# hilbertw/stereo_matching

Measured on AMD Instinct MI355X. Metric: Mpixel-disparities/s, 8-path SGM @ KITTI 1242×375 D=128; 1→8 GPU scaling, higher is better.
Workload: dtype f32; 1 GPU; config2: KITTI 1242x375 D=128, census 9x7 + Hamming cost + 8-path SGM + WTA/uniqueness/sub-pixel, left view (V=1), 1 pair per GPU; width=1242, height=375, max_disp=128, views=1, post_filter=False, lk_refine=False, sky_detect=False, launch=eager, pairs_per_gpu=1, global_batch=1, parallelism=1 pair on 1 GPU (single process: no process group, no gather)

## Files before the change

### stereo_matching_amd/csrc/sgm_cost.hip

```cpp
#include "sgm_device.h"

namespace sgm {


__device__ __forceinline__ int reflect101(int i, int n) {
    if (n == 1) return 0;
    i = i < 0 ? -i : i;
    return i >= n ? 2 * n - 2 - i : i;
}

constexpr int CT_TW = 64, CT_TH = 16, CT_RPT = CT_TH / 4;

template <int HH, int HWW>
__global__ __launch_bounds__(256) void census_kernel(const uint8_t *__restrict__ src0,
                                                     const uint8_t *__restrict__ src1, int rpitch,
                                                     int step, int H, int W, int blur,
                                                     uint64_t *__restrict__ ct0,
                                                     uint64_t *__restrict__ ct1) {
    const bool second = __builtin_amdgcn_workgroup_id_z() != 0;
    const uint8_t *__restrict__ src = second ? src1 : src0;
    uint64_t *__restrict__ ct = second ? ct1 : ct0;
    constexpr int TR = CT_TH + 2 * HH, TC = CT_TW + 2 * HWW;
    constexpr int RR = TR + 2, RC = TC + 2;
    constexpr int RAW_IT = (RR * RC + 255) / 256;
    __shared__ uint8_t tile[TR][TC];
    __shared__ uint8_t raw[RR][RC];
    const int x0 = bid_x() * CT_TW, y0 = bid_y() * CT_TH;
    const int t = tid_x();
    if (blur) {
        const int ylo = y0 - HH > 0 ? y0 - HH : 0, xlo = x0 - HWW > 0 ? x0 - HWW : 0;
        uint8_t v[RAW_IT];
#pragma unroll
        for (int u = 0; u < RAW_IT; ++u) {
            const int idx = u * 256 + t;
            const int ry = idx / RC, rx = idx - ry * RC;
            const int y = reflect101(clampi(ylo - 1 + ry, -1, H), H);
            const int x = reflect101(clampi(xlo - 1 + rx, -1, W), W);
            v[u] = idx < RR * RC ? src[(size_t)y * rpitch + (size_t)x * step] : 0;
        }
#pragma unroll
        for (int u = 0; u < RAW_IT; ++u) {
            const int idx = u * 256 + t;
            if (idx < RR * RC) (&raw[0][0])[idx] = v[u];
        }
        __syncthreads();
        for (int idx = t; idx < TR * TC; idx += 256) {
            const int ty = idx / TC, tx = idx - ty * TC;
            const int ry = clampi(y0 + ty - HH, 0, H - 1) - ylo;
            const int rx = clampi(x0 + tx - HWW, 0, W - 1) - xlo;
            constexpr int ky[3] = {70, 116, 70};
            int acc = 0;
#pragma unroll
            for (int r = 0; r < 3; ++r) {
                const uint8_t *row = &raw[ry + r][rx];
                acc += ky[r] * (82 * row[0] + 93 * row[1] + 82 * row[2]);
            }
            const int b = (acc + (1 << 15)) >> 16;
            tile[ty][tx] = (uint8_t)(b > 255 ? 255 : b);
        }
    } else {
        for (int idx = t; idx < TR * TC; idx += 256) {
            const int ty = idx / TC, tx = idx - ty * TC;
            const int y = clampi(y0 + ty - HH, 0, H - 1), x = clampi(x0 + tx - HWW, 0, W - 1);
            tile[ty][tx] = src[(size_t)y * rpitch + (size_t)x * step];
        }
    }
    __syncthreads();
    const int tx = t & 63, r0 = wave_id() * CT_RPT;
    constexpr int NB = (2 * HH + 1) * (2 * HWW + 1) - 1;
    static_assert(NB <= 64, "census word");
    constexpr int NHI = NB > 32 ? NB - 32 : 0;
    int c[CT_RPT];
#pragma unroll
    for (int p = 0; p < CT_RPT; ++p) c[p] = tile[r0 + p + HH][tx + HWW];
    unsigned hi[CT_RPT], lo[CT_RPT];
#pragma unroll
    for (int p = 0; p < CT_RPT; ++p) hi[p] = lo[p] = 0;
#pragma unroll
    for (int rr = 0; rr < CT_RPT + 2 * HH; ++rr) {
        int b[2 * HWW + 1];
#pragma unroll
        for (int dj = 0; dj <= 2 * HWW; ++dj) b[dj] = tile[r0 + rr][tx + dj];
#pragma unroll
        for (int p = 0; p < CT_RPT; ++p) {
            const int di = rr - p;
            if (di < 0 || di > 2 * HH) continue;
#pragma unroll
            for (int dj = 0; dj <= 2 * HWW; ++dj) {
                if (di == HH && dj == HWW) continue;
                const int k = di * (2 * HWW + 1) + dj - (di * (2 * HWW + 1) + dj > HH * (2 * HWW + 1) + HWW ? 1 : 0);
                const unsigned x = (unsigned)(c[p] - b[dj]);
                if (k < NHI) hi[p] = (hi[p] << 1) | (x >> 31);
                else lo[p] = (lo[p] << 1) | (x >> 31);
            }
        }
    }
    const int x = x0 + tx;
#pragma unroll
    for (int p = 0; p < CT_RPT; ++p) {
        const int y = y0 + r0 + p;
        if (y < H && x < W) ct[(size_t)y * W + x] = ((uint64_t)hi[p] << 32) | lo[p];
    }
}

hipError_t launch_census(const uint8_t *src, int pitch, Geom g, int blur, uint64_t *ct,
                         hipStream_t st, bool bm_rows, const uint8_t *src2, uint64_t *ct2) {
    dim3 grid((g.W + CT_TW - 1) / CT_TW, (g.H + CT_TH - 1) / CT_TH, src2 ? 2 : 1);
    const int rpitch = bm_rows ? pitch : pitch * g.scale;
    if (g.scale == 1)
        census_kernel<3, 4><<<grid, 256, 0, st>>>(src, src2, rpitch, 1, g.H, g.W, blur, ct, ct2);
    else
        census_kernel<1, 2><<<grid, 256, 0, st>>>(src, src2, rpitch, 2, g.H, g.W, blur, ct, ct2);
    return hipGetLastError();
}


__global__ __launch_bounds__(256) void ct_shift_kernel(const uint64_t *__restrict__ ctl,
                                                       const uint64_t *__restrict__ ctr,
                                                       uint64_t *__restrict__ ctl_s,
                                                       uint64_t *__restrict__ ctr_s, int W, int k) {
    const bool right = __builtin_amdgcn_workgroup_id_z() != 0;
    const uint64_t *__restrict__ src = right ? ctr : ctl;
    uint64_t *__restrict__ dst = right ? ctr_s : ctl_s;
    const int x = bid_x() * 256 + tid_x();
    if (dst == nullptr || x >= W) return;
    const size_t row = (size_t)bid_y() * W;
    const int xs = right ? (x - k > 0 ? x - k : 0) : (x + k < W - 1 ? x + k : W - 1);
    dst[row + x] = src[row + xs];
}

hipError_t launch_ct_shift(const uint64_t *ctl, const uint64_t *ctr, uint64_t *ctl_s, uint64_t *ctr_s,
                           int k, Geom g, hipStream_t st) {
    ct_shift_kernel<<<dim3((g.W + 255) / 256, g.H, 2), 256, 0, st>>>(ctl, ctr, ctl_s, ctr_s, g.W, k);
    return hipGetLastError();
}


constexpr int COSTH_MAX_LDS = 64 * 1024;

__device__ __forceinline__ void costh_store(float v, float *p) { __builtin_nontemporal_store(v, p); }
constexpr int COSTH_U = 8;

__host__ __device__ constexpr int costh_pad(int D, int scale) { return D / scale + 2 * COSTH_U; }

template <int VIEW, int WIN, bool SKY, bool FILTER, bool UNI, int DC = 0, int CK = 0>
__device__ __forceinline__ void cost_h_body(const uint64_t *__restrict__ ctl,
                                            const uint64_t *__restrict__ ctr,
                                            const uint8_t *__restrict__ sky, int sky_pitch, int H,
                                            int W, int D, int scale, int R,
                                            float *__restrict__ out, int blk, unsigned char *smem,
                                            int ck_ns = 0) {
    static_assert(CK == 0 || (WIN == 5 && FILTER), "checkpoints of the 5-wide filter");
    const int P = costh_pad(D, scale), RS = W + 2 * P;
    constexpr int NS = UNI ? 1 : 2;
    uint64_t *sl = reinterpret_cast<uint64_t *>(smem);
    uint64_t *sr = sl + (UNI ? 0 : (size_t)R * RS);
    uint8_t *ss = reinterpret_cast<uint8_t *>(sl + (size_t)NS * R * RS);
    const int row0 = blk * R;
    for (int idx = tid_x(); idx < R * RS; idx += R * D) {
        const int r = idx / RS, jp = idx - r * RS, i = row0 + r;
        const int j = clampi(jp - P, 0, W - 1);
        if (i < H) {
            if (!UNI || VIEW == 1) sl[idx] = ctl[(size_t)i * W + j];
            if (!UNI || VIEW == 0) sr[idx] = ctr[(size_t)i * W + j];
            if (SKY) ss[idx] = sky[(size_t)i * sky_pitch + j];
        }
    }
    __syncthreads();
    const int r = UNI ? uniform(tid_x() / D) : tid_x() / D, d = tid_x() - r * D;
    const int i = row0 + r;
    if (i >= H) return;
    const int ds = d / scale;
    const uint64_t *cl = sl + (size_t)r * RS + P + (VIEW == 1 ? ds : 0);
    const uint64_t *cr = sr + (size_t)r * RS + P - (VIEW == 0 ? ds : 0);
    const uint64_t *cu = (VIEW == 0 ? ctl : ctr) + (size_t)i * W;
    const uint8_t *sk = ss + (size_t)r * RS + P;
    float *o = out + (CK ? (size_t)i * ck_ns * 3 * D : (size_t)i * W * D) + d;
    const size_t DS = DC ? (size_t)DC : (size_t)D;

    auto word_l = [&](int j) { return UNI && VIEW == 0 ? cu[j < W - 1 ? j : W - 1] : cl[j]; };
    auto word_r = [&](int j) { return UNI && VIEW == 1 ? cu[j < W - 1 ? j : W - 1] : cr[j]; };

    auto raw = [&](int j) -> float {
        const float c = hamming(word_l(j), word_r(j));
        if (SKY) {
            const float sv = d == 0 ? 0.0f : 999999.0f;
            return sk[j] == 255 ? sv : c;
        }
        return c;
    };

    if (!FILTER) {
        for (int j = 0; j < W; ++j) costh_store(raw(j), o + (size_t)j * DS);
        return;
    }
    constexpr int HALF = WIN / 2, LAG = WIN - HALF - 1, U = COSTH_U;
    float sum = 0.0f;
#pragma unroll
    for (int k = 0; k < WIN; ++k) sum += raw(k);
    if constexpr (CK == 0) {
#pragma unroll
        for (int p = 0; p < LAG; ++p) costh_store(raw(p), o + (size_t)p * DS);
    }
    const int T = W - 2 * HALF;
    float hist[LAG > 0 ? LAG : 1];
#pragma unroll
    for (int p = 0; p < LAG; ++p) hist[p] = raw(p);
    auto ck_store = [&](int p) {
        if constexpr (CK > 0) {
            if (p % CK == 0) {
                float *q = o + (size_t)(p / CK) * 3 * DS;
                q[0] = sum;
                q[DS] = hist[0];
                q[2 * DS] = hist[LAG - 1];
            }
        }
    };
    auto step = [&](int t, float rw) {
        ck_store(LAG + t);
        const float v = div_win<WIN>(sum);
        if constexpr (CK == 0) costh_store(v, o + (size_t)(LAG + t) * DS);
        sum += rw;
        float a;
        if constexpr (LAG == 0) {
            a = v;
        } else {
            a = hist[0];
#pragma unroll
            for (int p = 0; p + 1 < LAG; ++p) hist[p] = hist[p + 1];
            hist[LAG - 1] = v;
        }
        sum -= a;
    };
    int t = 0;
    float cur[U];
    if (T - 1 >= U) {
#pragma unroll
        for (int u = 0; u < U; ++u) cur[u] = raw(WIN + u);
    }
    for (; t + 2 * U <= T - 1; t += U) {
        uint64_t nl[U], nr[U];
        uint8_t nk[U];
#pragma unroll
        for (int u = 0; u < U; ++u) {
            const int j = WIN + t + U + u;
            nl[u] = word_l(j);
            nr[u] = word_r(j);
            if (SKY) nk[u] = sk[j];
        }
#pragma unroll
        for (int u = 0; u < U; ++u) step(t + u, cur[u]);
#pragma unroll
        for (int u = 0; u < U; ++u) {
            const float c = hamming(nl[u], nr[u]);
            if (SKY) cur[u] = nk[u] == 255 ? (d == 0 ? 0.0f : 999999.0f) : c;
            else cur[u] = c;
        }
    }
    if (t + U <= T - 1) {
#pragma unroll
        for (int u = 0; u < U; ++u) step(t + u, cur[u]);
        t += U;
    }
    for (; t < T - 1; ++t) step(t, raw(WIN + t));
    if constexpr (CK > 0) {
        if (T >= 1) ck_store(LAG + T - 1);
        return;
    }
    if (T >= 1) costh_store(div_win<WIN>(sum), o + (size_t)(LAG + T - 1) * DS);
    for (int p = LAG + T; p < W; ++p) costh_store(raw(p), o + (size_t)p * DS);
}

template <int VIEW, int WIN, bool SKY, bool FILTER, bool UNI, int DC>
__global__ __launch_bounds__(256) void cost_h_kernel(const uint64_t *__restrict__ ctl,
                                                     const uint64_t *__restrict__ ctr,
                                                     const uint8_t *__restrict__ sky,
                                                     int sky_pitch, int H, int W, int D, int scale,
                                                     int R, float *__restrict__ out) {
    extern __shared__ __attribute__((aligned(16))) unsigned char smem[];
    cost_h_body<VIEW, WIN, SKY, FILTER, UNI, DC>(ctl, ctr, sky, sky_pitch, H, W, D, scale, R, out,
                                             bid_x(), smem);
}

template <int WIN, bool SKY, bool FILTER, bool UNI, int DC>
__global__ __launch_bounds__(256) void cost_h2_kernel(const uint64_t *__restrict__ ctl,
                                                      const uint64_t *__restrict__ ctr,
                                                      const uint64_t *__restrict__ ctl_s,
                                                      const uint64_t *__restrict__ ctr_s,
                                                      const uint8_t *__restrict__ sky0,
                                                      const uint8_t *__restrict__ sky1,
                                                      int sky_pitch, int H, int W, int D, int scale,
                                                      int R, float *__restrict__ out0,
                                                      float *__restrict__ out1) {
    extern __shared__ __attribute__((aligned(16))) unsigned char smem[];
    if (__builtin_amdgcn_workgroup_id_z() == 0)
        cost_h_body<0, WIN, SKY, FILTER, UNI, DC>(ctl, ctr_s, sky0, sky_pitch, H, W, D, scale, R, out0,
                                              bid_x(), smem);
    else
        cost_h_body<1, WIN, SKY, FILTER, UNI, DC>(ctl_s, ctr, sky1, sky_pitch, H, W, D, scale, R, out1,
                                              bid_x(), smem);
}

template <int VIEW, int WIN, bool SKY, bool FILTER>
__global__ __launch_bounds__(256) void cost_h_global_kernel(const uint64_t *__restrict__ ctl,
                                                            const uint64_t *__restrict__ ctr,
                                                            const uint8_t *__restrict__ sky,
                                                            int sky_pitch, int H, int W, int D,
                                                            int scale, float *__restrict__ out) {
    const int rows_per_block = 256 / D;
    const int r = tid_x() / D, d = tid_x() - r * D;
    const int i = bid_x() * rows_per_block + r;
    if (i >= H) return;
    const uint64_t *cl = ctl + (size_t)i * W;
    const uint64_t *cr = ctr + (size_t)i * W;
    const uint8_t *sk = SKY ? sky + (size_t)i * sky_pitch : nullptr;
    const int ds = d / scale;
    float *o = out + (size_t)i * W * D + d;
    auto raw = [&](int j) -> float {
        if (SKY && sk[j] == 255) return d == 0 ? 0.0f : 999999.0f;
        const uint64_t a = VIEW == 0 ? cl[j] : cl[min(j + ds, W - 1)];
        const uint64_t b = VIEW == 0 ? cr[max(j - ds, 0)] : cr[j];
        return hamming(a, b);
    };
    if (!FILTER) {
        for (int j = 0; j < W; ++j) costh_store(raw(j), o + (size_t)j * D);
        return;
    }
    constexpr int HALF = WIN / 2, LAG = WIN - HALF - 1;
    float sum = 0.0f;
#pragma unroll
    for (int k = 0; k < WIN; ++k) sum += raw(k);
#pragma unroll
    for (int p = 0; p < LAG; ++p) costh_store(raw(p), o + (size_t)p * D);
    const int T = W - 2 * HALF;
    float o1 = 0.0f, o2 = 0.0f;
    for (int t = 0; t < T; ++t) {
        const float v = div_win<WIN>(sum);
        costh_store(v, o + (size_t)(LAG + t) * D);
        if (t == T - 1) break;
        sum += raw(WIN + t);
        float a;
        if (LAG == 0) a = v;
        else if (LAG == 1) a = t >= 1 ? o1 : raw(t);
        else a = t >= 2 ? o2 : raw(t);
        sum -= a;
        o2 = o1;
        o1 = v;
    }
    for (int p = LAG + T; p < W; ++p) costh_store(raw(p), o + (size_t)p * D);
}

static void costh_shape(Geom g, bool sky, bool &uni, int &R, size_t &smem) {
    const size_t rs = (size_t)(g.W + 2 * costh_pad(g.D, g.scale));
    uni = g.D >= 64 && rs * (16 + (sky ? 1 : 0)) > (size_t)COSTH_MAX_LDS;
    const size_t row_bytes = rs * ((uni ? 8 : 16) + (sky ? 1 : 0));
    R = (int)(COSTH_MAX_LDS / row_bytes);
    if (R > 256 / g.D) R = 256 / g.D;
    smem = (size_t)(R > 0 ? R : 0) * row_bytes;
}

template <int VIEW, int WIN, bool SKY, bool FILTER>
static void launch_cost_h_t(const uint64_t *ctl, const uint64_t *ctr, const uint8_t *sky,
                            int sky_pitch, Geom g, float *out, hipStream_t st) {
    bool uni;
    int R;
    size_t smem;
    costh_shape(g, SKY, uni, R, smem);
    if (R >= 1) {
        if (uni)
            cost_h_kernel<VIEW, WIN, SKY, FILTER, true, 0><<<dim3((g.H + R - 1) / R), R * g.D, smem, st>>>(
                ctl, ctr, sky, sky_pitch, g.H, g.W, g.D, g.scale, R, out);
        else if (g.D == 128)
            cost_h_kernel<VIEW, WIN, SKY, FILTER, false, 128><<<dim3((g.H + R - 1) / R), R * g.D, smem, st>>>(
                ctl, ctr, sky, sky_pitch, g.H, g.W, g.D, g.scale, R, out);
        else
            cost_h_kernel<VIEW, WIN, SKY, FILTER, false, 0><<<dim3((g.H + R - 1) / R), R * g.D, smem, st>>>(
                ctl, ctr, sky, sky_pitch, g.H, g.W, g.D, g.scale, R, out);
    } else {
        const int rpb = 256 / g.D;
        cost_h_global_kernel<VIEW, WIN, SKY, FILTER><<<dim3((g.H + rpb - 1) / rpb), 256, 0, st>>>(
            ctl, ctr, sky, sky_pitch, g.H, g.W, g.D, g.scale, out);
    }
}

template <int VIEW, int WIN>
static void launch_cost_h_w(const uint64_t *ctl, const uint64_t *ctr, const uint8_t *sky,
                            int sky_pitch, int filter, Geom g, float *out, hipStream_t st) {
    if (sky) {
        if (filter) launch_cost_h_t<VIEW, WIN, true, true>(ctl, ctr, sky, sky_pitch, g, out, st);
        else launch_cost_h_t<VIEW, WIN, true, false>(ctl, ctr, sky, sky_pitch, g, out, st);
    } else {
        if (filter) launch_cost_h_t<VIEW, WIN, false, true>(ctl, ctr, sky, sky_pitch, g, out, st);
        else launch_cost_h_t<VIEW, WIN, false, false>(ctl, ctr, sky, sky_pitch, g, out, st);
    }
}

template <int WIN, bool SKY, bool FILTER>
static hipError_t launch_cost_h2_t(const uint64_t *ctl, const uint64_t *ctr, const uint64_t *ctl_s,
                                   const uint64_t *ctr_s, const uint8_t *sky0, const uint8_t *sky1,
                                   int sky_pitch, Geom g, float *out0, float *out1, hipStream_t st) {
    bool uni;
    int R;
    size_t smem;
    costh_shape(g, SKY, uni, R, smem);
    if (R < 1) return hipErrorInvalidValue;
    const dim3 grid((g.H + R - 1) / R, 1, 2);
    if (uni)
        cost_h2_kernel<WIN, SKY, FILTER, true, 0><<<grid, R * g.D, smem, st>>>(
            ctl, ctr, ctl_s, ctr_s, sky0, sky1, sky_pitch, g.H, g.W, g.D, g.scale, R, out0, out1);
    else if (g.D == 128)
        cost_h2_kernel<WIN, SKY, FILTER, false, 128><<<grid, R * g.D, smem, st>>>(
            ctl, ctr, ctl_s, ctr_s, sky0, sky1, sky_pitch, g.H, g.W, g.D, g.scale, R, out0, out1);
    else
        cost_h2_kernel<WIN, SKY, FILTER, false, 0><<<grid, R * g.D, smem, st>>>(
            ctl, ctr, ctl_s, ctr_s, sky0, sky1, sky_pitch, g.H, g.W, g.D, g.scale, R, out0, out1);
    return hipGetLastError();
}

bool cost_h2_supported(Geom g, bool sky) {
    bool uni;
    int R;
    size_t smem;
    costh_shape(g, sky, uni, R, smem);
    return R >= 1;
}

hipError_t launch_cost_h2(const uint64_t *ctl, const uint64_t *ctr, const uint64_t *ctl_s,
                          const uint64_t *ctr_s, const uint8_t *sky0, const uint8_t *sky1,
                          int sky_pitch, Geom g, float *out0, float *out1, hipStream_t st) {
    if ((sky0 == nullptr) != (sky1 == nullptr)) return hipErrorInvalidValue;
    if (sky0) {
        if (g.scale == 1) return launch_cost_h2_t<5, true, true>(ctl, ctr, ctl_s, ctr_s, sky0, sky1, sky_pitch, g, out0, out1, st);
        return launch_cost_h2_t<2, true, true>(ctl, ctr, ctl_s, ctr_s, sky0, sky1, sky_pitch, g, out0, out1, st);
    }
    if (g.scale == 1) return launch_cost_h2_t<5, false, true>(ctl, ctr, ctl_s, ctr_s, sky0, sky1, sky_pitch, g, out0, out1, st);
    return launch_cost_h2_t<2, false, true>(ctl, ctr, ctl_s, ctr_s, sky0, sky1, sky_pitch, g, out0, out1, st);
}

template <int VIEW, bool UNI>
__device__ __forceinline__ void cost_ck_body(const uint64_t *__restrict__ ctl,
                                             const uint64_t *__restrict__ ctr, int H, int W, int D,
                                             int R, float *__restrict__ out, int blk,
                                             unsigned char *smem, int ns) {
    constexpr int U = kVStripNC;
    const int P = costh_pad(D, 1), RS = W + 2 * P;
    constexpr int NS = UNI ? 1 : 2;
    uint64_t *sl = reinterpret_cast<uint64_t *>(smem);
    uint64_t *sr = sl + (UNI ? 0 : (size_t)R * RS);
    const int row0 = blk * R;
    for (int idx = tid_x(); idx < R * RS; idx += R * D) {
        const int r = idx / RS, jp = idx - r * RS, i = row0 + r;
        const int j = clampi(jp - P, 0, W - 1);
        if (i < H) {
            if (!UNI || VIEW == 1) sl[idx] = ctl[(size_t)i * W + j];
            if (!UNI || VIEW == 0) sr[idx] = ctr[(size_t)i * W + j];
        }
    }
    (void)NS;
    __syncthreads();
    const int r = UNI ? uniform(tid_x() / D) : tid_x() / D, d = tid_x() - r * D;
    const int i = row0 + r;
    if (i >= H) return;
    const uint64_t *cl = sl + (size_t)r * RS + P + (VIEW == 1 ? d : 0);
    const uint64_t *cr = sr + (size_t)r * RS + P - (VIEW == 0 ? d : 0);
    const uint64_t *cu = (VIEW == 0 ? ctl : ctr) + (size_t)i * W;
#ifdef COSTCK_VLOAD
    if constexpr (UNI) {
        int z;
        asm volatile("v_mov_b32 %0, 0" : "=v"(z));
        cu += z;
    }
#endif
    float *o = out + (size_t)i * ns * 3 * D + d;
    auto wu = [&](int j) { return UNI ? cu[j] : (VIEW == 0 ? cl[j] : cr[j]); };
    auto ws = [&](int j) { return VIEW == 0 ? cr[j] : cl[j]; };
    auto raw = [&](int j) {
        j = min(j, W - 1);
        return VIEW == 0 ? hamming(wu(j), ws(j)) : hamming(ws(j), wu(j));
    };
    float sum = 0.0f;
#pragma unroll
    for (int k = 0; k < 5; ++k) sum += raw(k);
    float h0 = raw(0), h1 = raw(1);
    const int T = W - 4;
    auto step = [&](float rw) {
        const float v = div_win<5>(sum);
        sum += rw;
        sum -= h0;
        h0 = h1;
        h1 = v;
    };
    auto ck_store = [&](int s) {
        float *q = o + (size_t)s * 3 * D;
        q[0] = sum;
        q[D] = h0;
        q[2 * D] = h1;
    };
    auto gstep = [&](int t) {
        if ((t + 2) % U == 0) ck_store((t + 2) / U);
        if (t < T - 1) step(raw(t + 5));
    };
    int t = 0;
    for (; t < U - 2 && t < T; ++t) gstep(t);
    int b = 1;
    if (U * (b + 1) - 2 < T) {
        float cur[U];
#pragma unroll
        for (int u = 0; u < U; ++u) cur[u] = raw(U * b + 3 + u);
        for (; U * (b + 1) - 2 < T; ++b) {
            uint64_t nu[U], nw[U];
#pragma unroll
            for (int u = 0; u < U; ++u) {
                const int j = min(U * (b + 1) + 3 + u, W - 1);
                nu[u] = wu(j);
                nw[u] = ws(j);
            }
            __builtin_amdgcn_sched_barrier(0);
            ck_store(b);
#pragma unroll
            for (int u = 0; u < U; ++u) step(cur[u]);
            __builtin_amdgcn_sched_barrier(0);
#pragma unroll
            for (int u = 0; u < U; ++u) cur[u] = VIEW == 0 ? hamming(nu[u], nw[u]) : hamming(nw[u], nu[u]);
        }
        t = U * b - 2;
    }
    for (; t < T; ++t) gstep(t);
}

template <bool SKY, bool UNI, int DC>
__global__ __launch_bounds__(256) void cost_ck_kernel(const uint64_t *__restrict__ ctl,
                                                      const uint64_t *__restrict__ ctr,
                                                      const uint64_t *__restrict__ ctl_s,
                                                      const uint64_t *__restrict__ ctr_s,
                                                      const uint8_t *__restrict__ sky0,
                                                      const uint8_t *__restrict__ sky1, int sky_pitch,
                                                      int H, int W, int D, int R, float *__restrict__ out0,
                                                      float *__restrict__ out1, int dsi0, int dsi1, int ns) {
    extern __shared__ __attribute__((aligned(16))) unsigned char smem[];
    const bool z = __builtin_amdgcn_workgroup_id_z() != 0;
    if constexpr (!SKY) {
        if ((z ? dsi1 : dsi0) == 0) cost_ck_body<0, UNI>(ctl, ctr_s, H, W, D, R, z ? out1 : out0, bid_x(), smem, ns);
        else cost_ck_body<1, UNI>(ctl_s, ctr, H, W, D, R, z ? out1 : out0, bid_x(), smem, ns);
    } else if ((z ? dsi1 : dsi0) == 0) {
        cost_h_body<0, 5, SKY, true, UNI, DC, kVStripNC>(ctl, ctr_s, z ? sky1 : sky0, sky_pitch, H, W, D, 1, R,
                                                         z ? out1 : out0, bid_x(), smem, ns);
    } else {
        cost_h_body<1, 5, SKY, true, UNI, DC, kVStripNC>(ctl_s, ctr, z ? sky1 : sky0, sky_pitch, H, W, D, 1, R,
                                                         z ? out1 : out0, bid_x(), smem, ns);
    }
}

template <bool SKY>
static hipError_t launch_cost_ck_t(const uint64_t *ctl, const uint64_t *ctr, const uint64_t *ctl_s,
                                   const uint64_t *ctr_s, const uint8_t *sky0, const uint8_t *sky1,
                                   int sky_pitch, int dsi0, int dsi1, int nviews, Geom g, float *ck0,
                                   float *ck1, hipStream_t st) {
    bool uni;
    int R;
    size_t smem;
    costh_shape(g, SKY, uni, R, smem);
    if (R < 1 || g.scale != 1) return hipErrorInvalidValue;
    const dim3 grid((g.H + R - 1) / R, 1, nviews);
    const int ns = (int)vstrip_strips(g);
#define CK_ARGS ctl, ctr, ctl_s, ctr_s, sky0, sky1, sky_pitch, g.H, g.W, g.D, R, ck0, ck1, dsi0, dsi1, ns
    if (uni) cost_ck_kernel<SKY, true, 0><<<grid, R * g.D, smem, st>>>(CK_ARGS);
    else if (g.D == 128) cost_ck_kernel<SKY, false, 128><<<grid, R * g.D, smem, st>>>(CK_ARGS);
    else cost_ck_kernel<SKY, false, 0><<<grid, R * g.D, smem, st>>>(CK_ARGS);
#undef CK_ARGS
    return hipGetLastError();
}

hipError_t launch_cost_ck(const uint64_t *ctl, const uint64_t *ctr, const uint64_t *ctl_s,
                          const uint64_t *ctr_s, const uint8_t *sky0, const uint8_t *sky1,
                          int sky_pitch, int dsi0, int dsi1, int nviews, Geom g, float *ck0,
                          float *ck1, hipStream_t st) {
    if (nviews == 2 && (sky0 == nullptr) != (sky1 == nullptr)) return hipErrorInvalidValue;
    if (sky0) return launch_cost_ck_t<true>(ctl, ctr, ctl_s, ctr_s, sky0, sky1, sky_pitch, dsi0, dsi1, nviews, g, ck0, ck1, st);
    return launch_cost_ck_t<false>(ctl, ctr, ctl_s, ctr_s, sky0, sky1, sky_pitch, dsi0, dsi1, nviews, g, ck0, ck1, st);
}

hipError_t launch_cost_h(const uint64_t *ctl, const uint64_t *ctr, const uint8_t *sky,
                         int sky_pitch, int view, int filter, Geom g, float *out,
                         hipStream_t st) {
    if (view == 0) {
        if (g.scale == 1) launch_cost_h_w<0, 5>(ctl, ctr, sky, sky_pitch, filter, g, out, st);
        else launch_cost_h_w<0, 2>(ctl, ctr, sky, sky_pitch, filter, g, out, st);
    } else {
        if (g.scale == 1) launch_cost_h_w<1, 5>(ctl, ctr, sky, sky_pitch, filter, g, out, st);
        else launch_cost_h_w<1, 2>(ctl, ctr, sky, sky_pitch, filter, g, out, st);
    }
    return hipGetLastError();
}


__global__ __launch_bounds__(256) void copy_kernel(const float *__restrict__ in,
                                                   float *__restrict__ out, size_t n) {
    const size_t i = (size_t)bid_x() * 256 + tid_x();
    if (i < n) out[i] = in[i];
}

hipError_t launch_copy(const float *in, float *out, Geom g, hipStream_t st) {
    const size_t n = (size_t)g.W * g.D * g.H;
    copy_kernel<<<dim3((unsigned)((n + 255) / 256)), 256, 0, st>>>(in, out, n);
    return hipGetLastError();
}


}
```

Measured before the change: 80610 Mpixel-disparities/s.

## Specialize checkpoint cost kernel on D, vectorize uniform loads, zero unreached strips

The checkpoint cost kernel is now templated on a compile-time disparity count (128/256), so index math folds into constants. The uniform-row path loads kVStripNC census words as one aligned struct, and the loop walks pointers incrementally instead of recomputing indices. Checkpoint stores are written inline. A new routine zeroes the checkpoint entries of strips the scan never reaches, and an env var can force the uniform (global-load) path; both add a few extra stores and launch options.

New measurement: 80470 Mpixel-disparities/s. About the same (-0.2%).

```diff
diff --git a/stereo_matching_amd/csrc/sgm_cost.hip b/stereo_matching_amd/csrc/sgm_cost.hip
--- a/stereo_matching_amd/csrc/sgm_cost.hip
+++ b/stereo_matching_amd/csrc/sgm_cost.hip
@@ -142,6 +142,17 @@
 constexpr int COSTH_U = 8;
 
 __host__ __device__ constexpr int costh_pad(int D, int scale) { return D / scale + 2 * COSTH_U; }
+
+
+__device__ __forceinline__ void ck_zero_unreached(float *o, int W, int ns, size_t DS) {
+    const int first = (W >= 5 ? (W - 3) / kVStripNC : 0) + 1;
+    for (int s = 0; s < ns; s = s == 0 ? first : s + 1) {
+        float *q = o + (size_t)s * 3 * DS;
+        q[0] = 0.0f;
+        q[DS] = 0.0f;
+        q[2 * DS] = 0.0f;
+    }
+}
 
 template <int VIEW, int WIN, bool SKY, bool FILTER, bool UNI, int DC = 0, int CK = 0>
 __device__ __forceinline__ void cost_h_body(const uint64_t *__restrict__ ctl,
@@ -265,6 +276,7 @@
     for (; t < T - 1; ++t) step(t, raw(WIN + t));
     if constexpr (CK > 0) {
         if (T >= 1) ck_store(LAG + T - 1);
+        ck_zero_unreached(o, W, ck_ns, DS);
         return;
     }
     if (T >= 1) costh_store(div_win<WIN>(sum), o + (size_t)(LAG + T - 1) * DS);
@@ -437,12 +449,17 @@
     return launch_cost_h2_t<2, false, true>(ctl, ctr, ctl_s, ctr_s, sky0, sky1, sky_pitch, g, out0, out1, st);
 }
 
-template <int VIEW, bool UNI>
+struct alignas(8) CkWords {
+    uint64_t w[kVStripNC];
+};
+
+template <int VIEW, bool UNI, int DC>
 __device__ __forceinline__ void cost_ck_body(const uint64_t *__restrict__ ctl,
-                                             const uint64_t *__restrict__ ctr, int H, int W, int D,
+                                             const uint64_t *__restrict__ ctr, int H, int W, int Drt,
                                              int R, float *__restrict__ out, int blk,
                                              unsigned char *smem, int ns) {
     constexpr int U = kVStripNC;
+    const int D = DC ? DC : Drt;
     const int P = costh_pad(D, 1), RS = W + 2 * P;
     constexpr int NS = UNI ? 1 : 2;
     uint64_t *sl = reinterpret_cast<uint64_t *>(smem);
@@ -464,13 +481,6 @@
     const uint64_t *cl = sl + (size_t)r * RS + P + (VIEW == 1 ? d : 0);
     const uint64_t *cr = sr + (size_t)r * RS + P - (VIEW == 0 ? d : 0);
     const uint64_t *cu = (VIEW == 0 ? ctl : ctr) + (size_t)i * W;
-#ifdef COSTCK_VLOAD
-    if constexpr (UNI) {
-        int z;
-        asm volatile("v_mov_b32 %0, 0" : "=v"(z));
-        cu += z;
-    }
-#endif
     float *o = out + (size_t)i * ns * 3 * D + d;
     auto wu = [&](int j) { return UNI ? cu[j] : (VIEW == 0 ? cl[j] : cr[j]); };
     auto ws = [&](int j) { return VIEW == 0 ? cr[j] : cl[j]; };
@@ -507,25 +517,34 @@
         float cur[U];
 #pragma unroll
         for (int u = 0; u < U; ++u) cur[u] = raw(U * b + 3 + u);
-        for (; U * (b + 1) - 2 < T; ++b) {
-            uint64_t nu[U], nw[U];
-#pragma unroll
-            for (int u = 0; u < U; ++u) {
-                const int j = min(U * (b + 1) + 3 + u, W - 1);
-                nu[u] = wu(j);
-                nw[u] = ws(j);
+        const uint64_t *wsp = (VIEW == 0 ? cr : cl) + (U * (b + 1) + 3);
+        const uint64_t *wup = (VIEW == 0 ? cl : cr) + (U * (b + 1) + 3);
+        float *q = o + (size_t)b * 3 * D;
+        for (; U * (b + 1) - 2 < T; ++b, wsp += U, wup += U, q += 3 * D) {
+            CkWords nu;
+            uint64_t nw[U];
+            if constexpr (UNI) {
+                nu = *reinterpret_cast<const CkWords *>(cu + min(U * (b + 1) + 3, W - U));
+            } else {
+#pragma unroll
+                for (int u = 0; u < U; ++u) nu.w[u] = wup[u];
             }
+#pragma unroll
+            for (int u = 0; u < U; ++u) nw[u] = wsp[u];
             __builtin_amdgcn_sched_barrier(0);
-            ck_store(b);
+            q[0] = sum;
+            q[D] = h0;
+            q[2 * D] = h1;
 #pragma unroll
             for (int u = 0; u < U; ++u) step(cur[u]);
             __builtin_amdgcn_sched_barrier(0);
 #pragma unroll
-            for (int u = 0; u < U; ++u) cur[u] = VIEW == 0 ? hamming(nu[u], nw[u]) : hamming(nw[u], nu[u]);
+            for (int u = 0; u < U; ++u) cur[u] = VIEW == 0 ? hamming(nu.w[u], nw[u]) : hamming(nw[u], nu.w[u]);
         }
         t = U * b - 2;
     }
     for (; t < T; ++t) gstep(t);
+    ck_zero_unreached(o, W, ns, (size_t)D);
 }
 
 template <bool SKY, bool UNI, int DC>
@@ -540,8 +559,8 @@
     extern __shared__ __attribute__((aligned(16))) unsigned char smem[];
     const bool z = __builtin_amdgcn_workgroup_id_z() != 0;
     if constexpr (!SKY) {
-        if ((z ? dsi1 : dsi0) == 0) cost_ck_body<0, UNI>(ctl, ctr_s, H, W, D, R, z ? out1 : out0, bid_x(), smem, ns);
-        else cost_ck_body<1, UNI>(ctl_s, ctr, H, W, D, R, z ? out1 : out0, bid_x(), smem, ns);
+        if ((z ? dsi1 : dsi0) == 0) cost_ck_body<0, UNI, DC>(ctl, ctr_s, H, W, D, R, z ? out1 : out0, bid_x(), smem, ns);
+        else cost_ck_body<1, UNI, DC>(ctl_s, ctr, H, W, D, R, z ? out1 : out0, bid_x(), smem, ns);
     } else if ((z ? dsi1 : dsi0) == 0) {
         cost_h_body<0, 5, SKY, true, UNI, DC, kVStripNC>(ctl, ctr_s, z ? sky1 : sky0, sky_pitch, H, W, D, 1, R,
                                                          z ? out1 : out0, bid_x(), smem, ns);
@@ -561,12 +580,25 @@
     size_t smem;
     costh_shape(g, SKY, uni, R, smem);
     if (R < 1 || g.scale != 1) return hipErrorInvalidValue;
+    const char *fu = getenv("SGM_COSTCK_UNI");
+    if (!uni && g.D >= 64 && fu && atoi(fu) > 0) {
+        uni = true;
+        smem = (size_t)R * (g.W + 2 * costh_pad(g.D, g.scale)) * (8 + (SKY ? 1 : 0));
+    }
     const dim3 grid((g.H + R - 1) / R, 1, nviews);
     const int ns = (int)vstrip_strips(g);
 #define CK_ARGS ctl, ctr, ctl_s, ctr_s, sky0, sky1, sky_pitch, g.H, g.W, g.D, R, ck0, ck1, dsi0, dsi1, ns
-    if (uni) cost_ck_kernel<SKY, true, 0><<<grid, R * g.D, smem, st>>>(CK_ARGS);
-    else if (g.D == 128) cost_ck_kernel<SKY, false, 128><<<grid, R * g.D, smem, st>>>(CK_ARGS);
-    else cost_ck_kernel<SKY, false, 0><<<grid, R * g.D, smem, st>>>(CK_ARGS);
+#define CK_LAUNCH(UNI_, DC_) cost_ck_kernel<SKY, UNI_, DC_><<<grid, R * g.D, smem, st>>>(CK_ARGS)
+    if (uni) {
+        if (g.D == 256) CK_LAUNCH(true, 256);
+        else if (g.D == 128) CK_LAUNCH(true, 128);
+        else CK_LAUNCH(true, 0);
+    } else {
+        if (g.D == 256) CK_LAUNCH(false, 256);
+        else if (g.D == 128) CK_LAUNCH(false, 128);
+        else CK_LAUNCH(false, 0);
+    }
+#undef CK_LAUNCH
 #undef CK_ARGS
     return hipGetLastError();
 }
```
